# Zanue/EndoDAV

Hardware: AMD Instinct MI355X
Metric: depth frames/sec (518x518, T=8 clip) (higher is better)
Workload: dtype f32

## Files before the change

### endodav_amd/_lib.py

```python
from __future__ import annotations

import ctypes as C
import os
from typing import Optional

_HERE = os.path.dirname(os.path.abspath(__file__))
LIB_PATH = os.environ.get("EDV_LIB_PATH") or os.path.join(_HERE, "lib", "libendodav_hip.so")
ABI_VERSION = 12

LORA_TYPES = {"none": 0, "lora": 1, "dvlora": 2, "ssb": 3, "dash": 4}
ACT_NONE, ACT_GELU, ACT_RELU, ACT_SIGMOID, ACT_SIGMOID_NEG = 0, 1, 2, 3, 4


class EdvConfig(C.Structure):

    _fields_ = [
        ("abi_version", C.c_int32),
        ("embed_dim", C.c_int32),
        ("depth", C.c_int32),
        ("num_heads", C.c_int32),
        ("taps", C.c_int32 * 4),
        ("features", C.c_int32),
        ("out_channels", C.c_int32 * 4),
        ("image_h", C.c_int32),
        ("image_w", C.c_int32),
        ("num_frames", C.c_int32),
        ("pos_tokens", C.c_int32),
        ("lora_type", C.c_int32),
        ("lora_rank", C.c_int32),
        ("include_cls_token", C.c_int32),
        ("conv_head", C.c_int32),
        ("inv_sigmoid", C.c_int32),
        ("out_sigmoid", C.c_int32),
        ("temporal_lora", C.c_int32),
        ("dash_active", C.c_int32),
        ("use_clstoken", C.c_int32),
        ("residual_mask", C.c_uint32),
        ("use_bn", C.c_int32),
        ("pe_rope", C.c_int32),
    ]

# ... 43 lines not shown
    "edv_backward": (C.c_int, [C.c_void_p, C.c_uint64, _fp, C.POINTER(C.c_void_p), C.c_void_p]),
    "edv_grad_bind_flat": (C.c_int, [C.c_void_p, _i32, C.POINTER(C.c_char_p), C.POINTER(_i64), _fp, _i64, C.POINTER(_i64)]),
    "edv_grad": (C.c_int, [C.c_void_p, C.c_char_p, C.POINTER(C.c_void_p), C.POINTER(_i64)]),
    "edv_grad_copy": (C.c_int, [C.c_void_p, C.c_char_p, _fp, _i64, C.c_void_p]),
    "edv_attn_spatial_x6_workspace": (C.c_size_t, [_i32, _i32, _i32]),
    "edv_attn_spatial_x6": (C.c_int, [_fp, _fp, _i32, _i32, _i32, _fp, C.c_size_t, C.c_void_p]),
    "edv_attn_spatial_bwd_workspace": (C.c_size_t, [_i32, _i32, _i32]),
    "edv_attn_spatial_bwd": (C.c_int, [_fp, _fp, _fp, _fp, _fp, _fp, _i32, _i32, _i32, _fp, C.c_size_t, C.c_void_p]),
    "edv_layernorm_bwd": (C.c_int, [_fp, _fp, _fp, _fp, _i64, _i32, C.c_float, _i32, C.c_void_p]),
    "edv_ew_bwd": (C.c_int, [_fp, _fp, _fp, _fp, _i64, _i32, C.c_void_p]),
    "edv_geglu_bwd": (C.c_int, [_fp, _fp, _fp, _i64, _i32, C.c_void_p]),
    "edv_transpose_scale": (C.c_int, [_fp, _fp, _fp, _i32, _i32, C.c_void_p]),
    "edv_lora_grads_workspace": (C.c_size_t, [_i64, _i32, _i32, _i32]),
    "edv_lora_grads": (C.c_int, [_fp, _fp, _i64, _i32, _i32, _i32, _fp, _fp, _fp, _fp, C.c_float, _fp, _fp, C.c_size_t, _fp, _fp, _fp, _fp, C.c_void_p]),
    "edv_bilinear_bwd": (C.c_int, [_fp, _fp, _i32, _i32, _i32, _i32, _i32, _i32, _i32, C.c_void_p]),
    "edv_dot_channels_bwd": (C.c_int, [_fp, _fp, _fp, _fp, _fp, _fp, _i64, _i32, _i32, C.c_void_p]),
    "edv_conv3x3_wgrad_workspace": (C.c_size_t, [_i32, _i32, _i32, _i32, _i32]),
    "edv_conv3x3_wgrad": (C.c_int, [_fp, _fp, _fp, _i32, _i32, _i32, _i32, _i32, _fp, C.c_size_t, _i32, C.c_void_p]),
    "edv_colsum_workspace": (C.c_size_t, [_i32]),
    "edv_colsum_rows": (C.c_int, [_fp, _fp, _i64, _i32, _fp, C.c_size_t, _fp, _i32, C.c_void_p]),
    "edv_colsum_batch_workspace": (C.c_size_t, [_i32, C.POINTER(_i64), C.POINTER(_i32)]),
    "edv_colsum_batch": (C.c_int, [_i32, C.POINTER(C.c_void_p), C.POINTER(_i64), C.POINTER(_i64), C.POINTER(_i32), C.POINTER(_i32), C.POINTER(C.c_void_p),
                                   C.POINTER(C.c_void_p), C.POINTER(_i32), _fp, C.c_size_t, C.c_void_p]),
    "edv_groupnorm_bwd": (C.c_int, [_fp, _fp, _fp, _fp, _fp, _fp, _i32, _i32, _i32, _i32, _i32, C.c_void_p]),
    "edv_attn_temporal_bwd": (C.c_int, [_fp, _fp, _fp, _i32, _i32, _i32, _i32, _i32, C.c_void_p]),
    "edv_pack_conv3x3_bwd": (C.c_int, [_fp, _fp, _i32, _i32, C.c_void_p]),
    "edv_conv3x3_s2_bwd": (C.c_int, [_fp, _fp, _fp, _i32, _i32, _i32, _i32, _i32, C.c_void_p]),
    "edv_dilate2": (C.c_int, [_fp, _fp, _i32, _i32, _i32, _i32, C.c_void_p]),
    "edv_pixel_unshuffle": (C.c_int, [_fp, _fp, _i32, _i32, _i32, _i32, _i32, C.c_void_p]),
    "edv_attn_temporal": (C.c_int, [_fp, _fp, _i32, _i32, _i32, _i32, _i32, C.c_void_p]),
    "edv_groupnorm_workspace": (C.c_size_t, [_i32, _i32, _i32]),
    "edv_groupnorm": (C.c_int, [_fp, _fp, _fp, _fp, _fp, _i32, _i32, _i32, _i32, _f32, _fp, C.c_size_t, C.c_void_p]),
    "edv_geglu": (C.c_int, [_fp, _fp, _i64, _i32, C.c_void_p]),
    "edv_rope_qk": (C.c_int, [_fp, _fp, _i32, _i32, _i32, _i32, _i32, C.c_void_p]),
    "edv_trainer_loss_workspace": (C.c_size_t, [_i32, _i32, _i32]),
    "edv_trainer_loss": (C.c_int, [C.c_void_p, _i32, _i32, _i32, C.c_void_p, _fp, C.c_void_p, _fp, C.c_size_t, C.c_void_p]),
    "edv_debug_fill_lds": (C.c_int, [C.c_float, C.c_void_p]),
    "edv_bilinear": (C.c_int, [_fp, _fp, _i32, _i32, _i32, _i32, _i32, _i32, C.c_void_p]),
    "edv_dot_channels": (C.c_int, [_fp, _fp, _fp, _fp, _i64, _i32, _i32, C.c_void_p]),
    "edv_patchify": (C.c_int, [_fp, _fp, _i32, _i32, _i32, _i32, _i32, C.c_void_p]),
    "edv_bicubic_pos": (C.c_int, [_fp, _fp, _i32, _i32, _i32, _i32, _f64, _f64, C.c_void_p]),
    "edv_resize_bicubic": (C.c_int, [_fp, _fp, _i32, _i32, _i32, _i32, _i32, C.c_void_p]),
    "edv_stitch_workspace": (C.c_size_t, []),
    "edv_stitch_fit": (C.c_int, [_fp, _i32, _i32, _fp, _i32, _i32, _fp, _fp, C.c_size_t, C.c_void_p]),
    "edv_stitch_apply": (C.c_int, [_fp, _i32, _i32, _fp, _fp, _fp, _i32, _i32, C.c_void_p]),
    "edv_photometric_loss_workspace": (C.c_size_t, [_i32, _i32, _i32, _i32]),
    "edv_photometric_loss": (C.c_int, [_fp, C.POINTER(C.c_void_p), C.POINTER(_i32), C.POINTER(_i32), _i32, _i32, _i32, _i32, _fp, _fp, _fp, _fp, _f32, _f32, _f32,
                                       _fp, C.POINTER(C.c_void_p), _fp, C.c_size_t, C.c_void_p]),
    "edv_fold_lora": (C.c_int, [_fp, _fp, _fp, _fp, _fp, _f32, _fp, _i32, _i32, _i32, C.c_void_p]),
}


KERNEL_CLASSES = {"linear": 0, "conv3x3": 1, "attn_spatial": 2, "attn_temporal": 3, "layernorm": 4, "other": 5, "linear_encoder": 6,
                  "groupnorm": 7, "bilinear": 8, "geglu": 9, "dot_channels": 10, "patchify": 11, "attn_spatial_bwd": 12}
HBM_CLASSES = ("layernorm", "groupnorm", "bilinear", "geglu", "dot_channels", "patchify")


class EdvError(RuntimeError):
    pass


_lib: Optional[C.CDLL] = None


def load() -> C.CDLL:
    global _lib
# ... 2 lines not shown
    if not os.path.exists(LIB_PATH):
        raise EdvError(
            f"{LIB_PATH} is missing: build it with `make` (hipcc --offload-arch=gfx950) or "
            "`python -c 'import __graft_entry__ as g; g.build()'`.  There is no CPU fallback."
        )
    lib = C.CDLL(LIB_PATH)
    for name, (res, args) in SIGNATURES.items():
        fn = getattr(lib, name)
        fn.restype = res
        fn.argtypes = args
    got = lib.edv_abi_version()
    if got != ABI_VERSION:
        raise EdvError(f"libendodav_hip ABI {got} != binding ABI {ABI_VERSION}")
    _lib = lib
    return lib


def check(status: int, what: str = "") -> None:
    if status != 0:
        msg = load().edv_last_error()
        raise EdvError(f"{what}: {msg.decode() if msg else 'unknown error'}")


def ptr(t) -> int:
    return 0 if t is None else t.data_ptr()


class TrainerLossInputs(C.Structure):
    _fields_ = [("color", C.c_void_p * 4), ("color_nb", C.c_void_p * 2), ("K", C.c_void_p), ("invK", C.c_void_p), ("T", C.c_void_p * 2),
                ("refined", (C.c_void_p * 2) * 4), ("registration", (C.c_void_p * 2) * 4), ("transform", (C.c_void_p * 2) * 4), ("mask", C.c_void_p * 2),
                ("position", (C.c_void_p * 2) * 4), ("disp", C.c_void_p * 4), ("disp_h", C.c_int32 * 4), ("disp_w", C.c_int32 * 4)]


class TrainerLossWeights(C.Structure):
    _fields_ = [("disparity_smoothness", C.c_float), ("transform_constraint", C.c_float), ("transform_smoothness", C.c_float), ("depth_reproj", C.c_float),
                ("depth_flow", C.c_float), ("tune_temporal", C.c_int32), ("min_depth", C.c_float), ("max_depth", C.c_float)]


class TrainerLossGrads(C.Structure):
    _fields_ = [("disp", C.c_void_p * 4), ("refined", (C.c_void_p * 2) * 4), ("transform", (C.c_void_p * 2) * 4), ("K", C.c_void_p), ("invK", C.c_void_p),
                ("T", C.c_void_p * 2)]


def stream_ptr(device=None) -> int:
    import torch

    return torch.cuda.current_stream(device).cuda_stream
```

### endodav_amd/csrc/api.hip

```cpp
#include "../../include/endodav_hip.h"
#include <vector>

#include "ops.hpp"

using namespace edv;

extern "C" {

int edv_layernorm(const float *x_dev, const float *w_dev, const float *b_dev, float *y_dev, int64_t rows, int32_t dim, float eps,
                  const float *pe_dev, int32_t rows_per_frame, int32_t T, void *stream) {
    return layernorm(x_dev, identity_map(), w_dev, b_dev, y_dev, identity_map(), rows, dim, eps, pe_dev, rows_per_frame, T, (hipStream_t)stream);
}

size_t edv_gemm_workspace(void) { return gemm_workspace() * sizeof(float); }
int edv_gemm(const float *A_dev, const float *W_dev, float *C_dev, int64_t M, int32_t N, int32_t K, const float *bias_dev, int32_t act,
             const float *gamma_dev, const float *R_dev, float *workspace_dev, size_t workspace_bytes, void *stream) {
    GemmDesc g;
    g.A = A_dev; g.lda = K; g.W = W_dev; g.ldw = K; g.C = C_dev; g.ldc = N; g.M = M; g.N = N; g.K = K;
    g.bias = bias_dev; g.act = act; g.gamma = gamma_dev; g.R1 = R_dev; g.ldr1 = N;
    g.ws = workspace_dev; g.ws_floats = workspace_bytes / sizeof(float);
    EDV_CHECK(act >= ACT_NONE && act <= ACT_RELU, "act must be 0, 1 or 2");
    return gemm(g, (hipStream_t)stream);
}

size_t edv_gemm_x6_planes_bytes(int32_t N, int32_t K) { return N > 0 && K > 0 ? gemm_x6_planes_bytes(N, K) : 0; }

int edv_gemm_x6_split(const float *W_dev, void *planes_dev, int32_t N, int32_t K, void *stream) {
    return gemm_x6_split(W_dev, planes_dev, N, K, (hipStream_t)stream);
}

int edv_gemm_x6(const float *A_dev, const void *planes_dev, float *C_dev, int64_t M, int32_t N, int32_t K, const float *bias_dev, int32_t act,
                const float *gamma_dev, const float *R_dev, float *workspace_dev, size_t workspace_bytes, void *stream) {
    GemmDesc g;
// ... 139 lines not shown
    return groupnorm_bwd(x_dev, stats_dev, w_dev, dy_dev, sums_dev, dx_dev, F, P, C, groups, accumulate != 0, (hipStream_t)stream);
}
int edv_attn_temporal_bwd(const float *qkv_dev, const float *dout_dev, float *dqkv_dev, int32_t B, int32_t T, int32_t P, int32_t C, int32_t heads,
                          void *stream) {
    return attn_temporal_bwd(qkv_dev, dout_dev, dqkv_dev, B, T, P, C, heads, (hipStream_t)stream);
}
int edv_pack_conv3x3_bwd(const float *w_dev, float *wpacked_dev, int32_t Cout, int32_t Cin, void *stream) {
    return pack_conv3x3_bwd(w_dev, wpacked_dev, Cout, Cin, (hipStream_t)stream);
}
int edv_conv3x3_s2_bwd(const float *dy_dev, const float *wpacked_dev, float *dx_dev, int32_t F, int32_t H, int32_t W, int32_t Cin, int32_t Cout,
                       void *stream) {
    return conv3x3_s2_bwd(dy_dev, wpacked_dev, dx_dev, F, H, W, Cin, Cout, (hipStream_t)stream);
}
int edv_dilate2(const float *dy_dev, float *z_dev, int32_t F, int32_t H, int32_t W, int32_t C, void *stream) {
    return dilate2(dy_dev, z_dev, F, H, W, C, (hipStream_t)stream);
}
int edv_pixel_unshuffle(const float *dy_dev, float *A_dev, int32_t F, int32_t h, int32_t w, int32_t C, int32_t s, void *stream) {
    return pixel_unshuffle(dy_dev, A_dev, F, h, w, C, s, (hipStream_t)stream);
}

int edv_attn_temporal(const float *qkv_dev, float *out_dev, int32_t B, int32_t T, int32_t P, int32_t C, int32_t heads, void *stream) {
    return attn_temporal(qkv_dev, out_dev, B, T, P, C, heads, (hipStream_t)stream);
}

int edv_rope_qk(float *qkv_dev, const float *table_dev, int32_t B, int32_t T, int32_t P, int32_t C, int32_t transpose, void *stream) {
    return rope_qk(qkv_dev, table_dev, B, T, P, C, transpose != 0, (hipStream_t)stream);
}

size_t edv_groupnorm_workspace(int32_t F, int32_t P, int32_t C) { return groupnorm_workspace(F, P, C) * sizeof(float); }

int edv_groupnorm(const float *x_dev, const float *w_dev, const float *b_dev, float *y_dev, float *stats_dev, int32_t F, int32_t P, int32_t C,
                  int32_t groups, float eps, float *workspace_dev, size_t workspace_bytes, void *stream) {
    return groupnorm(x_dev, w_dev, b_dev, y_dev, stats_dev, F, P, C, groups, eps, (hipStream_t)stream, workspace_dev, workspace_bytes / sizeof(float));
}

namespace edv {
namespace {
__global__ __launch_bounds__(256) void fill_lds_kernel(float value, float *sink) {
    extern __shared__ float lds_all[];
    for (int i = threadIdx.x; i < 160 * 256; i += 256) lds_all[i] = value;
    __syncthreads();
    if (sink && lds_all[(threadIdx.x * 97) % (160 * 256)] != value) *sink = 1.f;
}
}
}
int edv_debug_fill_lds(float value, void *stream) {
    int dev = 0, cus = 0;
    EDV_HIP(hipGetDevice(&dev));
    EDV_HIP(hipDeviceGetAttribute(&cus, hipDeviceAttributeMultiprocessorCount, dev));
    EDV_HIP(hipFuncSetAttribute(reinterpret_cast<const void *>(edv::fill_lds_kernel), hipFuncAttributeMaxDynamicSharedMemorySize, 160 * 1024));
    EDV_LAUNCH(edv::fill_lds_kernel, dim3((unsigned)(8 * cus)), dim3(256), 160 * 1024, (hipStream_t)stream, value, (float *)nullptr);
    EDV_LAUNCH_OK();
    return 0;
}

int edv_geglu(const float *x_dev, float *y_dev, int64_t M, int32_t inner, void *stream) { return geglu(x_dev, y_dev, M, inner, (hipStream_t)stream); }

int edv_bilinear(const float *x_dev, float *y_dev, int32_t F, int32_t H, int32_t W, int32_t C, int32_t OH, int32_t OW, void *stream) {
    return bilinear(x_dev, y_dev, F, H, W, C, OH, OW, ACT_NONE, (hipStream_t)stream);
}

int edv_dot_channels(const float *x_dev, const float *w_dev, const float *b_dev, float *y_dev, int64_t M, int32_t C, int32_t act, void *stream) {
    EDV_CHECK(act == ACT_NONE || act == ACT_RELU || act == ACT_SIGMOID || act == ACT_SIGMOID_NEG, "act must be 0, 2, 3 or 4");
    return dot_channels(x_dev, w_dev, b_dev, y_dev, M, C, act, (hipStream_t)stream);
}

// ... 76 lines not shown
```

### endodav_amd/csrc/engine_forward.hip

```cpp
#include "engine.hpp"

namespace {

struct OnStream {
    Run &r;
    const hipStream_t st;
    float *const skws;
    const int F;
    OnStream(Run &run, hipStream_t s, float *ws) : r(run), st(run.st), skws(run.skws), F(run.F) { r.st = s; r.skws = ws; }
    ~OnStream() { r.st = st; r.skws = skws; r.F = F; }
};

struct Forward : Run {
    using Run::Run;
    std::string rb_suffix;
    int enc_F = 0, enc_f0 = 0;
    bool stagger_record = false;
    float *tap[4], *tapcls[4] = {nullptr, nullptr, nullptr, nullptr}, *pj[4], *lv[4], *rn[4], *path[5], *readout = nullptr, *fbias = nullptr;

    int pos_table(const float **out) {
        const float *pos;
        EDV_TRY(param("pretrained.pos_embed", &pos, 3));
        const int Npos = cfg.pos_tokens - 1;
        const int npatch = ntok - 1;
        if (npatch == Npos && cfg.image_h == cfg.image_w) {
            *out = pos;
            return 0;
        }
        const int S = (int)std::lround(std::sqrt((double)Npos));
        EDV_CHECK(S * S == Npos, "pos_embed grid is not square");
        float *tab;
        EDV_TRY(wsbuf("pos_eff", (size_t)ntok * D, &tab));
        const double sh = ((double)ph + 0.1) / std::sqrt((double)Npos), sw = ((double)pw + 0.1) / std::sqrt((double)Npos);
        EDV_CHECK((int)std::floor(S * sh) == ph && (int)std::floor(S * sw) == pw, "pos-embed resample size mismatch");
        if (c0) EDV_TRY(copy_f32(pos, tab, D, st));
        EDV_TRY(bicubic_pos(pos + D, tab + (size_t)c0 * D, S, D, ph, pw, (float)(1.0 / sh), (float)(1.0 / sw), st));
        c->launches += 2;
        *out = tab;
        return 0;
    }

    int snapshot(const std::string &name, const float *src, size_t n) {
        if (c->capture) {
            float *dst;
            EDV_TRY(wsbuf("stage." + name, n, &dst));
            EDV_TRY(copy_f32(src, dst, (long long)n, st));
            c->stages[name] = {dst, n};
        }
        return 0;
    }

    int motion_module(int m, float *x, int P, int C, const float *extra = nullptr) {
        const std::string p = "head.motion_modules." + std::to_string(m) + ".temporal_transformer";
        const std::string tb = p + ".transformer_blocks.0";
        const long long M = (long long)F * P;
        float *gn, *h, *hn, *qkv3, *att, *ff1, *ff2, *stats;
        const std::string sc_ = m == 1 ? "mmb." : "mm.";
        const std::string tg = c->train ? "mm" + std::to_string(m) + "." : sc_;
        float *hs[4];
        const float *xin = x;
        EDV_TRY(wsbuf(sc_ + "gn", (size_t)M * C, &gn));
        EDV_TRY(wsbuf(tg + "h", (size_t)M * C, &h));
        hs[0] = hs[1] = hs[2] = hs[3] = h;
        if (c->train) {
            float *xc;
            EDV_TRY(wsbuf(tg + "xin", (size_t)M * C, &xc));
            EDV_TRY(copy_f32(x, xc, M * C, st));
            xin = xc;
            for (int k = 1; k < 4; ++k) EDV_TRY(wsbuf(tg + "h" + std::to_string(k), (size_t)M * C, &hs[k]));
        }
        EDV_TRY(wsbuf(sc_ + "hn", (size_t)M * C, &hn));
        EDV_TRY(wsbuf(sc_ + "att", (size_t)M * C, &att));
        EDV_TRY(wsbuf(tg + "ff1", (size_t)M * 8 * C, &ff1));
        EDV_TRY(wsbuf(c->train ? tg + "ff2" : sc_ + "ff2", (size_t)M * 4 * C, &ff2));
        EDV_TRY(wsbuf(tg + "stats", (size_t)F * 32 * 2, &stats));
        const float *w, *b;
        EDV_TRY(param(p + ".norm.weight", &w));
        EDV_TRY(param(p + ".norm.bias", &b));
        float *gnpart = nullptr;
        size_t gnpart_n = 0;
        if ((long long)F * P * C >= 1500000ll) {
            gnpart_n = groupnorm_workspace(F, P, C);
            EDV_TRY(wsbuf(sc_ + "gnpart", gnpart_n, &gnpart));
        }
        {
            HbmScope b_(c, KC_GROUPNORM, st, 8.0 * (double)M * C);
            EDV_TRY(groupnorm(xin, w, b, gn, stats, F, P, C, 32, 1e-6f, st, gnpart, gnpart_n));
        }
// ... 612 lines not shown
```

### endodav_amd/csrc/norms.hip

```cpp
#include <cstdlib>

#include "ops.hpp"

namespace edv {
namespace {

using f32x4 = __attribute__((ext_vector_type(4))) float;
constexpr int LN_MAXV = 4;

template <int R, int NV>
__global__ __launch_bounds__(256) void layernorm_kernel(const float *__restrict__ x, RowMap in_map, const float *__restrict__ w,
                                                         const float *__restrict__ b, float *y, RowMap out_map, long long rows,
                                                         int dim, float eps, const float *__restrict__ pe, int rows_per_frame, int T, int act,
                                                         int accumulate) {
    const int lane = threadIdx.x & 63;
    const long long row0 = ((long long)blockIdx.x * 4 + (threadIdx.x >> 6)) * R;
    if (row0 >= rows) return;
    const int nv = dim >> 2;
    f32x4 v[R][NV];
    float s[R];
#pragma unroll
    for (int k = 0; k < R; ++k) {
        const long long row = row0 + k < rows ? row0 + k : rows - 1;
        const float *xr = x + in_map(row) * dim;
// ... 182 lines not shown
    EDV_CHECK(x && w && b && y, "null operand");
    EDV_CHECK(act == ACT_NONE || act == ACT_GELU, "layernorm act must be none or gelu");
    EDV_CHECK(rows > 0, "empty problem");
    EDV_CHECK(dim % 4 == 0 && dim <= 256 * LN_MAXV, "dim must be a multiple of 4 and <= 1024");
    EDV_CHECK(!pe || (rows_per_frame > 0 && T > 0), "pe needs rows_per_frame and T");
    static const int forced = [] {
        const char *e = getenv("EDV_LN_ROWS");
        return e ? atoi(e) : 0;
    }();
    int R = 1;
    if (forced == 1 || forced == 2 || forced == 4) R = forced;
    if (dim > 512 && R > 2) R = 2;
    const long long blocks = (rows + 4 * R - 1) / (4 * R);
    EDV_CHECK(blocks < (1ll << 31), "grid");
    const int rpf = rows_per_frame > 0 ? rows_per_frame : 1, TT = T > 0 ? T : 1, acc = accumulate ? 1 : 0;
#define EDV_LN_LAUNCH(RR, NVV)                                                                                                                  \
    EDV_LAUNCH((layernorm_kernel<RR, NVV>), dim3((unsigned)blocks), dim3(256), 0, st, x, in_map, w, b, y, out_map, rows, dim, eps, pe, rpf, TT, \
                       act, acc)
    if (dim <= 512) {
        if (R == 4) EDV_LN_LAUNCH(4, 2);
        else if (R == 2) EDV_LN_LAUNCH(2, 2);
        else EDV_LN_LAUNCH(1, 2);
    } else {
        if (R == 2) EDV_LN_LAUNCH(2, 4);
        else EDV_LN_LAUNCH(1, 4);
    }
#undef EDV_LN_LAUNCH
    EDV_LAUNCH_OK();
    return 0;
}

size_t groupnorm_workspace(int F, int P, int C) { return (size_t)F * ((P + GN_ROWS - 1) / GN_ROWS) * 2 * C; }

int groupnorm(const float *x, const float *w, const float *b, float *y, float *stats, int F, int P, int C, int groups, float eps, hipStream_t st, float *part,
              size_t part_floats) {
    EDV_CHECK(x && w && b && y && stats, "null operand");
    EDV_CHECK(F > 0 && P > 0 && C > 0 && groups > 0 && C % groups == 0 && C % 4 == 0, "shape");
    EDV_CHECK(F <= 65535, "grid");
    const int nch = (P + GN_ROWS - 1) / GN_ROWS;
    if (part && C <= 1024 && nch <= 65535) {
        EDV_CHECK(groupnorm_workspace(F, P, C) <= part_floats && (uintptr_t)part % 16 == 0, "groupnorm workspace too small (groupnorm_workspace)");
        EDV_LAUNCH(groupnorm_partial_kernel, dim3(nch, F), dim3(256), 0, st, x, part, P, C, nch);
        EDV_LAUNCH_OK();
        EDV_LAUNCH(groupnorm_finish_kernel, dim3(groups, F), dim3(64), 0, st, part, stats, P, C, groups, nch, eps);
        EDV_LAUNCH_OK();
    } else {
        EDV_LAUNCH(groupnorm_stats_kernel, dim3(groups, F), dim3(256), 0, st, x, stats, P, C, groups, eps);
        EDV_LAUNCH_OK();
    }
    EDV_CHECK(C <= 1024, "groupnorm: at most 1024 channels");
    const int rpp = 256 / (C >> 2);
    int chunks = (P + 4 * rpp - 1) / (4 * rpp);
    chunks = chunks < 1 ? 1 : (chunks > 2048 ? 2048 : chunks);
    EDV_LAUNCH(groupnorm_apply_kernel, dim3((unsigned)chunks, (unsigned)F), dim3(256), 0, st, x, stats, w, b, y, P, C, groups);
    EDV_LAUNCH_OK();
    return 0;
}

}
```

### endodav_amd/csrc/ops.hpp

```cpp
#pragma once
#include "common.hpp"

namespace edv {

enum { ACT_NONE = 0, ACT_GELU = 1, ACT_RELU = 2, ACT_SIGMOID = 3, ACT_SIGMOID_NEG = 4 };
enum { LOAD_DENSE = 0, LOAD_CONV3 = 1 };
enum { STORE_ROWS = 0, STORE_SHUFFLE = 1 };

struct GemmDesc {
    const float *A = nullptr;
    int lda = 0;
    RowMap a_map{0, 0, 0};
    const float *W = nullptr;
    int ldw = 0;
    float *C = nullptr;
    int ldc = 0;
    RowMap c_map{0, 0, 0};
    long long M = 0;
    int N = 0, K = 0;
    const float *bias = nullptr;
    int act = ACT_NONE;
    const float *gamma = nullptr;
    const float *R1 = nullptr;
    int ldr1 = 0;
// ... 9 lines not shown
    int geglu = 0;
    int ps_s = 0, ps_C = 0, ps_h = 0, ps_w = 0;
    float *ws = nullptr;
    size_t ws_floats = 0;
    const void *Wx6 = nullptr;
};
int gemm(const GemmDesc &d, hipStream_t st);
size_t gemm_x6_planes_bytes(int N, int K);
int gemm_x6_split(const float *W, void *planes, int N, int K, hipStream_t st);
bool gemm_x6_supported(const GemmDesc &d);
int gemm_x6(const GemmDesc &d, hipStream_t st);
size_t gemm_workspace();
size_t gemm_counter_bytes();
bool gemm_dma_supported(const GemmDesc &d);
bool gemm_geglu_supported(const GemmDesc &d);
int pack_geglu(const float *w, const float *b, float *wi, float *bi, int N, int K, hipStream_t st);
int gemm_dma(const GemmDesc &d, hipStream_t st);
bool conv_dma_supported(const GemmDesc &d);
int conv_dma(const GemmDesc &d, hipStream_t st);
const char *gemm_kernel_name(const GemmDesc &d);

size_t attn_spatial_workspace(int F, int N, int heads, bool x6 = false);
int attn_spatial(const float *qkv, float *out, int F, int N, int heads, float *ws, size_t ws_floats, hipStream_t st, float *lse = nullptr, bool x6 = false);
size_t attn_spatial_bwd_workspace(int F, int N, int heads);
int attn_spatial_bwd(const float *qkv, const float *out, const float *dout, const float *lse, float *delta, float *dqkv, int F, int N, int heads, float *ws,
                     size_t ws_floats, hipStream_t st);
int attn_temporal(const float *qkv, float *out, int B, int T, int P, int C, int heads, hipStream_t st);
int geglu(const float *x, float *y, long long M, int inner, hipStream_t st);
int rope_qk(float *qkv, const float *table, int B, int T, int P, int C, bool transpose, hipStream_t st);

int layernorm(const float *x, RowMap in_map, const float *w, const float *b, float *y, RowMap out_map, long long rows, int dim,
              float eps, const float *pe, int rows_per_frame, int T, hipStream_t st, int act = ACT_NONE, bool accumulate = false);
size_t groupnorm_workspace(int F, int P, int C);
int groupnorm(const float *x, const float *w, const float *b, float *y, float *stats, int F, int P, int C, int groups, float eps, hipStream_t st,
              float *part = nullptr, size_t part_floats = 0);

int patchify(const float *x, float *cols, int F, int H, int W, int ih, int iw, hipStream_t st, int ld = 588)  ;
int bilinear(const float *x, float *y, int F, int H, int W, int C, int OH, int OW, int act, hipStream_t st, const float *add = nullptr);
int dot_channels(const float *x, const float *w, const float *b, float *y, long long M, int C, int act, hipStream_t st);
int cls_rows(const float *cls, const float *pos, float *tokens, int F, int ntok, int D, hipStream_t st);
int sigmoid_inplace(float *x, long long n, hipStream_t st);
int resize_bicubic(const float *x, float *y, int NP, int H, int W, int OH, int OW, hipStream_t st);
size_t stitch_workspace();
int stitch_fit(const float *disp, int ih, int iw, const float *tail, int fh, int fw, float *st, void *ws, size_t ws_bytes, hipStream_t stream);
int stitch_apply(const float *disp, int ih, int iw, const float *st, float *tail, float *out_new, int fh, int fw, hipStream_t stream);
int bicubic_pos(const float *grid, float *out, int S, int D, int oh, int ow, float scale_h, float scale_w, hipStream_t st);

int pack_conv3x3(const float *w, float *out, int Cout, int Cin, hipStream_t st);
int pack_convT(const float *w, float *wout, const float *b, float *bout, int Cin, int Cout, int s, hipStream_t st);
int copy_f32(const float *src, float *dst, long long n, hipStream_t st);
int fold_lora(const float *W, const float *A, const float *B, const float *U, const float *V, float scale, float *out, int nout, int nin,
              int r, hipStream_t st);
int fold_ssb(const float *W, const float *a, const float *b, float *out, int nout, int nin, hipStream_t st);
int fold_bn(float *w, const float *b, const float *gamma, const float *beta, const float *mean, const float *var, float eps, float *bout, int nout, int K,
            hipStream_t st);
int fold_dash(const float *Utop, const float *idx, const float *Vtop, float *inout, int nout, int nin, int r, hipStream_t st);

int layernorm_bwd(const float *x, RowMap xmap, const float *w, const float *dy, RowMap dymap, float *dx, RowMap dxmap, long long rows, int dim, float eps,
                  bool accumulate, hipStream_t st);
int ew_bwd(const float *d, const float *src, const float *add, float *out, long long n, int mode, hipStream_t st);
int sigmoid_bwd(const float *g, const float *s, float *out, long long n, hipStream_t st);
int geglu_bwd(const float *x, const float *dy, float *dx, long long M, int inner, hipStream_t st);
int transpose_scale(const float *W, int ldw, const float *gamma, float *Wt, int N, int K, hipStream_t st);
int skinny_xwt(const float *X, long long M, int K, int ldx, const float *Wr, int r, float *T, hipStream_t st);
constexpr int TALL_SPLITS = 64;
size_t tall_tn_workspace(int N, int r);
int tall_tn(const float *Y, int ldy, const float *T, long long M, int N, int r, float scale, const float *rowscale, float *part, float *out, hipStream_t st);
int lora_grad_finalize(const float *dBp, const float *dApT, const float *A, const float *Bm, const float *U, const float *V, float *dA, float *dB, float *dU,
// ... 73 lines not shown
```

### include/endodav_hip.h

```cpp
#ifndef ENDODAV_HIP_H
#define ENDODAV_HIP_H

#include <stddef.h>
#include <stdint.h>

#ifdef __cplusplus
extern "C" {
#endif

#define EDV_ABI_VERSION 12

enum edv_lora_type { EDV_LORA_NONE = 0, EDV_LORA_LORA = 1, EDV_LORA_DVLORA = 2, EDV_LORA_SSB = 3, EDV_LORA_DASH = 4 };

typedef struct edv_config {
    int32_t abi_version;
    int32_t embed_dim;
    int32_t depth;
    int32_t num_heads;
    int32_t taps[4];
    int32_t features;
    int32_t out_channels[4];
    int32_t image_h, image_w;
    int32_t num_frames;
    int32_t pos_tokens;
    int32_t lora_type;
    int32_t lora_rank;
    int32_t include_cls_token;
    int32_t conv_head;
    int32_t inv_sigmoid;
    int32_t out_sigmoid;
    int32_t temporal_lora;
    int32_t dash_active;
    int32_t use_clstoken;
    uint32_t residual_mask;
    int32_t use_bn;
    int32_t pe_rope;
} edv_config;

typedef struct edv_ctx edv_ctx;

int edv_abi_version(void);
const char *edv_last_error(void);
int edv_create(const edv_config *cfg, edv_ctx **out);
// ... 31 lines not shown
size_t edv_gemm_x6_planes_bytes(int32_t N, int32_t K);
int edv_gemm_x6_split(const float *W_dev, void *planes_dev, int32_t N, int32_t K, void *stream);
int edv_gemm_x6(const float *A_dev, const void *planes_dev, float *C_dev, int64_t M, int32_t N, int32_t K, const float *bias_dev, int32_t act,
                const float *gamma_dev, const float *R_dev, float *workspace_dev, size_t workspace_bytes, void *stream);

int edv_pack_geglu(const float *w_dev, const float *b_dev, float *wi_dev, float *bi_dev, int32_t N, int32_t K, void *stream);
int edv_gemm_geglu(const float *A_dev, const float *Wi_dev, const float *bi_dev, float *C_dev, int64_t M, int32_t N, int32_t K, void *stream);

int edv_conv3x3(const float *x_dev, const float *wpacked_dev, const float *bias_dev, float *y_dev, int32_t F, int32_t H, int32_t W,
                int32_t Cin, int32_t Cout, int32_t stride, int32_t pre_relu, int32_t post_relu, const float *R1_dev,
                const float *R2_dev, void *stream);
int edv_conv3x3_ws(const float *x_dev, const float *wpacked_dev, const float *bias_dev, float *y_dev, int32_t F, int32_t H, int32_t W,
                   int32_t Cin, int32_t Cout, int32_t stride, int32_t pre_relu, int32_t post_relu, const float *R1_dev,
                   const float *R2_dev, float *workspace_dev, size_t workspace_bytes, void *stream);
int edv_pack_conv3x3(const float *w_dev, float *wpacked_dev, int32_t Cout, int32_t Cin, void *stream);

size_t edv_attn_spatial_workspace(int32_t F, int32_t N, int32_t heads);
int edv_attn_spatial(const float *qkv_dev, float *out_dev, int32_t F, int32_t N, int32_t heads, float *workspace_dev,
                     size_t workspace_bytes, float *lse_dev, void *stream);
size_t edv_attn_spatial_x6_workspace(int32_t F, int32_t N, int32_t heads);
int edv_attn_spatial_x6(const float *qkv_dev, float *out_dev, int32_t F, int32_t N, int32_t heads, float *workspace_dev, size_t workspace_bytes,
                        void *stream);
size_t edv_attn_spatial_bwd_workspace(int32_t F, int32_t N, int32_t heads);
int edv_attn_spatial_bwd(const float *qkv_dev, const float *out_dev, const float *dout_dev, const float *lse_dev, float *delta_dev,
                         float *dqkv_dev, int32_t F, int32_t N, int32_t heads, float *workspace_dev, size_t workspace_bytes, void *stream);

int edv_attn_temporal(const float *qkv_dev, float *out_dev, int32_t B, int32_t T, int32_t P, int32_t C, int32_t heads, void *stream);

int edv_rope_qk(float *qkv_dev, const float *table_dev, int32_t B, int32_t T, int32_t P, int32_t C, int32_t transpose, void *stream);

size_t edv_groupnorm_workspace(int32_t F, int32_t P, int32_t C);
int edv_groupnorm(const float *x_dev, const float *w_dev, const float *b_dev, float *y_dev, float *stats_dev ,
                  int32_t F, int32_t P, int32_t C, int32_t groups, float eps, float *workspace_dev, size_t workspace_bytes, void *stream);

int edv_geglu(const float *x_dev, float *y_dev, int64_t M, int32_t inner, void *stream);

int edv_debug_fill_lds(float value, void *stream);

int edv_bilinear(const float *x_dev, float *y_dev, int32_t F, int32_t H, int32_t W, int32_t C, int32_t OH, int32_t OW, void *stream);

int edv_dot_channels(const float *x_dev, const float *w_dev, const float *b_dev, float *y_dev, int64_t M, int32_t C, int32_t act, void *stream);

int edv_patchify(const float *x_dev, float *cols_dev, int32_t F, int32_t H, int32_t W, int32_t ih, int32_t iw, void *stream);

int edv_conv_transpose(const float *x_dev, const float *w_dev, const float *b_dev, float *wpack_dev, float *bpack_dev, float *y_dev, int32_t F, int32_t h,
              int32_t w, int32_t C, int32_t s, void *stream);

int edv_bicubic_pos(const float *grid_dev, float *out_dev, int32_t S, int32_t D, int32_t oh, int32_t ow, double scale_h, double scale_w, void *stream);

int edv_resize_bicubic(const float *x_dev, float *y_dev, int32_t planes, int32_t H, int32_t W, int32_t OH, int32_t OW, void *stream);

size_t edv_stitch_workspace(void);
int edv_stitch_fit(const float *disp_dev, int32_t ih, int32_t iw, const float *tail_dev, int32_t fh, int32_t fw, float *st_dev, void *workspace_dev,
                   size_t workspace_bytes, void *stream);
int edv_stitch_apply(const float *disp_dev, int32_t ih, int32_t iw, const float *st_dev, float *tail_dev, float *new_dev, int32_t fh, int32_t fw,
                     void *stream);

int edv_fold_lora(const float *W_dev, const float *A_dev, const float *B_dev, const float *U_dev, const float *V_dev, float scale, float *out_dev,
                  int32_t nout, int32_t nin, int32_t r, void *stream);

int edv_set_train(edv_ctx *ctx, int32_t on);
int edv_set_grad_scope(edv_ctx *ctx, int32_t encoder_factors, int32_t temporal_factors, int32_t head_convs, int32_t residual_blocks);
int edv_set_bias_grads(edv_ctx *ctx, int32_t encoder_biases, int32_t head_biases);
int edv_generation(const edv_ctx *ctx, uint64_t *generation);
int edv_backward(edv_ctx *ctx, uint64_t generation, const float *disp0_dev, const float *const grad_disp_dev[4], void *stream);
int edv_grad_bind_flat(edv_ctx *ctx, int32_t n, const char *const *names, const int64_t *numels, float *flat_dev, int64_t flat_floats,
// ... 71 lines not shown
```

Before: 1077.

## Fuse temporal motion module into a single MFMA kernel per pixel tile

Adds a fused HIP kernel that runs the whole temporal transformer motion module (groupnorm apply, proj_in, two temporal attention blocks with layernorm and positional encoding, GEGLU feed-forward, proj_out and residual) for 64-channel, 8-head blocks in registers using fp32 MFMA. Only groupnorm statistics stay in a separate launch, which removes many intermediate global-memory round trips and kernel launches in inference. It is enabled by default for non-training runs without RoPE, and adds a new ABI entry point. The cost is heavy register use and redundant weight loads per wave.

After: 1082, median of 6. Within noise of the previous version (+0.5%).

```diff
diff --git a/endodav_amd/_lib.py b/endodav_amd/_lib.py
--- a/endodav_amd/_lib.py
+++ b/endodav_amd/_lib.py
@@ -6,7 +6,7 @@
 
 _HERE = os.path.dirname(os.path.abspath(__file__))
 LIB_PATH = os.environ.get("EDV_LIB_PATH") or os.path.join(_HERE, "lib", "libendodav_hip.so")
-ABI_VERSION = 12
+ABI_VERSION = 13
 
 LORA_TYPES = {"none": 0, "lora": 1, "dvlora": 2, "ssb": 3, "dash": 4}
 ACT_NONE, ACT_GELU, ACT_RELU, ACT_SIGMOID, ACT_SIGMOID_NEG = 0, 1, 2, 3, 4
@@ -116,6 +116,9 @@
     "edv_groupnorm_workspace": (C.c_size_t, [_i32, _i32, _i32]),
     "edv_groupnorm": (C.c_int, [_fp, _fp, _fp, _fp, _fp, _i32, _i32, _i32, _i32, _f32, _fp, C.c_size_t, C.c_void_p]),
     "edv_geglu": (C.c_int, [_fp, _fp, _i64, _i32, C.c_void_p]),
+    "edv_motion_module_fused_supported": (C.c_int, [_i32, _i32, _i32]),
+    "edv_motion_module_fused_workspace": (C.c_size_t, [_i32, _i32, _i32]),
+    "edv_motion_module_fused": (C.c_int, [_fp, _fp, C.c_void_p, _fp, C.c_size_t, _i32, _i32, _i32, C.c_void_p]),
     "edv_rope_qk": (C.c_int, [_fp, _fp, _i32, _i32, _i32, _i32, _i32, C.c_void_p]),
     "edv_trainer_loss_workspace": (C.c_size_t, [_i32, _i32, _i32]),
     "edv_trainer_loss": (C.c_int, [C.c_void_p, _i32, _i32, _i32, C.c_void_p, _fp, C.c_void_p, _fp, C.c_size_t, C.c_void_p]),
@@ -184,6 +187,13 @@
                 ("position", (C.c_void_p * 2) * 4), ("disp", C.c_void_p * 4), ("disp_h", C.c_int32 * 4), ("disp_w", C.c_int32 * 4)]
 
 
+class MotionParams(C.Structure):
+    _fields_ = [("gn_w", C.c_void_p), ("gn_b", C.c_void_p), ("proj_in_w", C.c_void_p), ("proj_in_b", C.c_void_p), ("ln_w", C.c_void_p * 2),
+                ("ln_b", C.c_void_p * 2), ("pe", C.c_void_p * 2), ("qkv_w", C.c_void_p * 2), ("out_w", C.c_void_p * 2), ("out_b", C.c_void_p * 2),
+                ("ffn_w", C.c_void_p), ("ffn_b", C.c_void_p), ("ff0_w", C.c_void_p), ("ff0_b", C.c_void_p), ("ff2_w", C.c_void_p), ("ff2_b", C.c_void_p),
+                ("proj_out_w", C.c_void_p), ("proj_out_b", C.c_void_p)]
+
+
 class TrainerLossWeights(C.Structure):
     _fields_ = [("disparity_smoothness", C.c_float), ("transform_constraint", C.c_float), ("transform_smoothness", C.c_float), ("depth_reproj", C.c_float),
                 ("depth_flow", C.c_float), ("tune_temporal", C.c_int32), ("min_depth", C.c_float), ("max_depth", C.c_float)]
diff --git a/endodav_amd/csrc/api.hip b/endodav_amd/csrc/api.hip
--- a/endodav_amd/csrc/api.hip
+++ b/endodav_amd/csrc/api.hip
@@ -1,4 +1,5 @@
 #include "../../include/endodav_hip.h"
+#include <cstring>
 #include <vector>
 
 #include "ops.hpp"
@@ -204,6 +205,21 @@
 int edv_groupnorm(const float *x_dev, const float *w_dev, const float *b_dev, float *y_dev, float *stats_dev, int32_t F, int32_t P, int32_t C,
                   int32_t groups, float eps, float *workspace_dev, size_t workspace_bytes, void *stream) {
     return groupnorm(x_dev, w_dev, b_dev, y_dev, stats_dev, F, P, C, groups, eps, (hipStream_t)stream, workspace_dev, workspace_bytes / sizeof(float));
+}
+
+int edv_motion_module_fused_supported(int32_t T, int32_t C, int32_t heads) { return motion_fused_supported(T, C, heads) ? 1 : 0; }
+
+size_t edv_motion_module_fused_workspace(int32_t B, int32_t T, int32_t P) {
+    return B > 0 && T > 0 && P > 0 ? motion_module_fused_workspace(B * T, P) * sizeof(float) : 0;
+}
+
+int edv_motion_module_fused(float *x_dev, const float *extra_dev, const edv_motion_params *params, float *workspace_dev, size_t workspace_bytes, int32_t B,
+                            int32_t T, int32_t P, void *stream) {
+    EDV_CHECK(params, "null argument");
+    static_assert(sizeof(edv_motion_params) == sizeof(MotionFusedParams), "edv_motion_params mirrors MotionFusedParams");
+    MotionFusedParams q;
+    memcpy(&q, params, sizeof(q));
+    return motion_module_fused(x_dev, extra_dev, q, workspace_dev, workspace_bytes / sizeof(float), B, T, P, (hipStream_t)stream);
 }
 
 namespace edv {
diff --git a/endodav_amd/csrc/engine_forward.hip b/endodav_amd/csrc/engine_forward.hip
--- a/endodav_amd/csrc/engine_forward.hip
+++ b/endodav_amd/csrc/engine_forward.hip
@@ -50,10 +50,42 @@
         return 0;
     }
 
+    int motion_module_fused_path(const std::string &p, const std::string &tb, int m, float *x, int P, const float *extra) {
+        MotionFusedParams q;
+        EDV_TRY(param(p + ".norm.weight", &q.gn_w));
+        EDV_TRY(param(p + ".norm.bias", &q.gn_b));
+        EDV_TRY(param(p + ".proj_in.weight", &q.proj_in_w));
+        EDV_TRY(param(p + ".proj_in.bias", &q.proj_in_b));
+        for (int a = 0; a < 2; ++a) {
+            const std::string ab = tb + ".attention_blocks." + std::to_string(a), nb = tb + ".norms." + std::to_string(a);
+            EDV_TRY(param(nb + ".weight", &q.ln_w[a]));
+            EDV_TRY(param(nb + ".bias", &q.ln_b[a]));
+            EDV_TRY(param(ab + ".pos_encoder.pe", &q.pe[a]));
+            EDV_TRY(packedw(ab + ".qkv", &q.qkv_w[a]));
+            EDV_TRY(param(ab + ".to_out.0.weight", &q.out_w[a]));
+            EDV_TRY(param(ab + ".to_out.0.bias", &q.out_b[a]));
+        }
+        EDV_TRY(param(tb + ".ff_norm.weight", &q.ffn_w));
+        EDV_TRY(param(tb + ".ff_norm.bias", &q.ffn_b));
+        EDV_TRY(param(tb + ".ff.net.0.proj.weight", &q.ff0_w));
+        EDV_TRY(param(tb + ".ff.net.0.proj.bias", &q.ff0_b));
+        EDV_TRY(lin_w(tb + ".ff.net.2", &q.ff2_w));
+        EDV_TRY(param(tb + ".ff.net.2.bias", &q.ff2_b));
+        EDV_TRY(param(p + ".proj_out.weight", &q.proj_out_w));
+        EDV_TRY(param(p + ".proj_out.bias", &q.proj_out_b));
+        const size_t nws = motion_module_fused_workspace(F, P);
+        float *ws;
+        EDV_TRY(wsbuf((m == 1 ? "mmb." : "mm.") + std::string("fused"), nws, &ws));
+        Bracket b_(c, KC_ATTN_TEMPORAL, st);
+        return motion_module_fused(x, extra, q, ws, nws, B, T, P, st, &c->launches);
+    }
+
     int motion_module(int m, float *x, int P, int C, const float *extra = nullptr) {
         const std::string p = "head.motion_modules." + std::to_string(m) + ".temporal_transformer";
         const std::string tb = p + ".transformer_blocks.0";
         const long long M = (long long)F * P;
+        static const bool mm_fused = env_flag("EDV_MM_FUSED", true);
+        if (mm_fused && !c->train && !cfg.pe_rope && motion_fused_supported(T, C, 8)) return motion_module_fused_path(p, tb, m, x, P, extra);
         float *gn, *h, *hn, *qkv3, *att, *ff1, *ff2, *stats;
         const std::string sc_ = m == 1 ? "mmb." : "mm.";
         const std::string tg = c->train ? "mm" + std::to_string(m) + "." : sc_;
diff --git a/endodav_amd/csrc/motion_fused.hip b/endodav_amd/csrc/motion_fused.hip
--- /dev/null
+++ b/endodav_amd/csrc/motion_fused.hip
@@ -0,0 +1,223 @@
+#include "ops.hpp"
+
+namespace edv {
+namespace {
+
+using f32x4 = __attribute__((ext_vector_type(4))) float;
+using f32x16 = __attribute__((ext_vector_type(16))) float;
+
+__device__ __forceinline__ f32x4 ld4(const float *p) { return *reinterpret_cast<const f32x4 *>(p); }
+
+template <int KB>
+__device__ __forceinline__ f32x16 lin32(f32x16 acc, const float *__restrict__ wr, const f32x16 (&xin)[KB]) {
+#pragma unroll
+    for (int kb = 0; kb < KB; ++kb) {
+#pragma unroll
+        for (int q = 0; q < 4; ++q) {
+            const f32x4 w4 = ld4(wr + 32 * kb + 8 * q);
+#pragma unroll
+            for (int e = 0; e < 4; ++e) acc = __builtin_amdgcn_mfma_f32_32x32x2f32(w4[e], xin[kb][4 * q + e], acc, 0, 0, 0);
+        }
+    }
+    return acc;
+}
+
+__device__ __forceinline__ f32x16 feat32(const float *__restrict__ v) {
+    f32x16 o;
+#pragma unroll
+    for (int q = 0; q < 4; ++q) {
+        const f32x4 b4 = ld4(v + 8 * q);
+#pragma unroll
+        for (int e = 0; e < 4; ++e) o[4 * q + e] = b4[e];
+    }
+    return o;
+}
+
+__device__ __forceinline__ float hsum16(const f32x16 v) {
+    return (((v[0] + v[1]) + (v[2] + v[3])) + ((v[4] + v[5]) + (v[6] + v[7]))) + (((v[8] + v[9]) + (v[10] + v[11])) + ((v[12] + v[13]) + (v[14] + v[15])));
+}
+
+__device__ __forceinline__ void ln64(const f32x16 (&in)[2], f32x16 (&out)[2], const float *__restrict__ w, const float *__restrict__ b,
+                                     const float *__restrict__ pe, int h, float eps) {
+    float s = hsum16(in[0]) + hsum16(in[1]);
+    s += __shfl_xor(s, 32, 64);
+    const float mean = s * (1.0f / 64.0f);
+    const f32x16 d0 = in[0] - mean, d1 = in[1] - mean;
+    float q = hsum16(d0 * d0) + hsum16(d1 * d1);
+    q += __shfl_xor(q, 32, 64);
+    const float rstd = rsqrtf(q * (1.0f / 64.0f) + eps);
+    out[0] = d0 * rstd * feat32(w + 4 * h) + feat32(b + 4 * h);
+    out[1] = d1 * rstd * feat32(w + 32 + 4 * h) + feat32(b + 32 + 4 * h);
+    if (pe) {
+        out[0] += feat32(pe);
+        out[1] += feat32(pe + 32);
+    }
+}
+
+template <int T>
+__device__ __forceinline__ f32x16 attn_block(const f32x16 q, const f32x16 k, const f32x16 v, float scale) {
+    float s[4][T];
+#pragma unroll
+    for (int j = 0; j < T; ++j) {
+#pragma unroll
+        for (int hh = 0; hh < 4; ++hh) {
+            float kk[4];
+#pragma unroll
+            for (int e = 0; e < 4; ++e) kk[e] = j ? __shfl_xor(k[4 * hh + e], j, 64) : k[4 * hh + e];
+            s[hh][j] = (q[4 * hh] * kk[0] + q[4 * hh + 1] * kk[1]) + (q[4 * hh + 2] * kk[2] + q[4 * hh + 3] * kk[3]);
+        }
+    }
+    float inv[4];
+#pragma unroll
+    for (int hh = 0; hh < 4; ++hh) {
+        float mx = -INFINITY;
+#pragma unroll
+        for (int j = 0; j < T; ++j) {
+            s[hh][j] = (s[hh][j] + __shfl_xor(s[hh][j], 32, 64)) * scale;
+            mx = fmaxf(mx, s[hh][j]);
+        }
+        float sum = 0.f;
+#pragma unroll
+        for (int j = 0; j < T; ++j) {
+            s[hh][j] = expf(s[hh][j] - mx);
+            sum += s[hh][j];
+        }
+        inv[hh] = 1.0f / sum;
+    }
+    f32x16 o;
+#pragma unroll
+    for (int i = 0; i < 16; ++i) o[i] = s[i >> 2][0] * v[i];
+#pragma unroll
+    for (int j = 1; j < T; ++j) {
+#pragma unroll
+        for (int i = 0; i < 16; ++i) o[i] += s[i >> 2][j] * __shfl_xor(v[i], j, 64);
+    }
+#pragma unroll
+    for (int i = 0; i < 16; ++i) o[i] *= inv[i >> 2];
+    return o;
+}
+
+template <int T>
+__global__ __launch_bounds__(256, 2) void motion_fused_kernel(float *x, const float *__restrict__ extra, const MotionFusedParams p,
+                                                            const float *__restrict__ stats, int P, int tiles_per_clip, int ntiles) {
+    constexpr int PPT = 32 / T;
+    constexpr int C = 64;
+    const int lane = threadIdx.x & 63, n = lane & 31, h = lane >> 5;
+    const int tile = blockIdx.x * 4 + (threadIdx.x >> 6);
+    if (tile >= ntiles) return;
+    const int b = tile / tiles_per_clip, tc = tile - b * tiles_per_clip;
+    const int t = n % T;
+    int pix = tc * PPT + n / T;
+    const bool valid = pix < P;
+    if (!valid) pix = P - 1;
+    const long long frame = (long long)b * T + t;
+    const long long off = (frame * P + pix) * C + 4 * h;
+
+    f32x16 a[2];
+#pragma unroll
+    for (int q = 0; q < 8; ++q) {
+        const f32x4 v = ld4(x + off + 8 * q);
+        const f32x4 ms = ld4(stats + (frame * 32 + 4 * q + 2 * h) * 2);
+        const f32x4 gw = ld4(p.gn_w + 8 * q + 4 * h), gb = ld4(p.gn_b + 8 * q + 4 * h);
+        a[q >> 2][4 * (q & 3) + 0] = (v[0] - ms[0]) * (ms[1] * gw[0]) + gb[0];
+        a[q >> 2][4 * (q & 3) + 1] = (v[1] - ms[0]) * (ms[1] * gw[1]) + gb[1];
+        a[q >> 2][4 * (q & 3) + 2] = (v[2] - ms[2]) * (ms[3] * gw[2]) + gb[2];
+        a[q >> 2][4 * (q & 3) + 3] = (v[3] - ms[2]) * (ms[3] * gw[3]) + gb[3];
+    }
+    const int wrow = n * C + 4 * h;
+    f32x16 hres[2], hn[2];
+#pragma unroll
+    for (int ob = 0; ob < 2; ++ob) hres[ob] = lin32<2>(feat32(p.proj_in_b + 32 * ob + 4 * h), p.proj_in_w + 32 * ob * C + wrow, a);
+
+    const float scale = 0.35355339059327373f;
+#pragma unroll 1
+    for (int ab = 0; ab < 2; ++ab) {
+        ln64(hres, hn, p.ln_w[ab], p.ln_b[ab], p.pe[ab] + t * C + 4 * h, h, 1e-5f);
+        const float *__restrict__ wq = p.qkv_w[ab] + wrow;
+        f32x16 o[2];
+#pragma unroll
+        for (int blk = 0; blk < 2; ++blk) {
+            f32x16 z = {0.f, 0.f, 0.f, 0.f, 0.f, 0.f, 0.f, 0.f, 0.f, 0.f, 0.f, 0.f, 0.f, 0.f, 0.f, 0.f};
+            const f32x16 qq = lin32<2>(z, wq + (32 * blk) * C, hn);
+            const f32x16 kk = lin32<2>(z, wq + (64 + 32 * blk) * C, hn);
+            const f32x16 vv = lin32<2>(z, wq + (128 + 32 * blk) * C, hn);
+            o[blk] = attn_block<T>(qq, kk, vv, scale);
+        }
+#pragma unroll
+        for (int ob = 0; ob < 2; ++ob) hres[ob] += lin32<2>(feat32(p.out_b[ab] + 32 * ob + 4 * h), p.out_w[ab] + 32 * ob * C + wrow, o);
+    }
+
+    ln64(hres, hn, p.ffn_w, p.ffn_b, nullptr, h, 1e-5f);
+    f32x16 y[2];
+#pragma unroll
+    for (int ob = 0; ob < 2; ++ob) y[ob] = feat32(p.ff2_b + 32 * ob + 4 * h);
+#pragma unroll 1
+    for (int c = 0; c < 8; ++c) {
+        const f32x16 val = lin32<2>(feat32(p.ff0_b + 32 * c + 4 * h), p.ff0_w + (32 * c) * C + wrow, hn);
+        const f32x16 gate = lin32<2>(feat32(p.ff0_b + 256 + 32 * c + 4 * h), p.ff0_w + (256 + 32 * c) * C + wrow, hn);
+        f32x16 g[1];
+#pragma unroll
+        for (int i = 0; i < 16; ++i) g[0][i] = val[i] * gelu_erf(gate[i]);
+#pragma unroll
+        for (int ob = 0; ob < 2; ++ob) y[ob] = lin32<1>(y[ob], p.ff2_w + (32 * ob + n) * (4 * C) + 32 * c + 4 * h, g);
+    }
+#pragma unroll
+    for (int ob = 0; ob < 2; ++ob) hres[ob] += y[ob];
+
+#pragma unroll
+    for (int ob = 0; ob < 2; ++ob) y[ob] = lin32<2>(feat32(p.proj_out_b + 32 * ob + 4 * h), p.proj_out_w + 32 * ob * C + wrow, hres);
+    if (!valid) return;
+#pragma unroll
+    for (int q = 0; q < 8; ++q) {
+        f32x4 r = ld4(x + off + 8 * q);
+        if (extra) r += ld4(extra + off + 8 * q);
+#pragma unroll
+        for (int e = 0; e < 4; ++e) r[e] += y[q >> 2][4 * (q & 3) + e];
+        *reinterpret_cast<f32x4 *>(x + off + 8 * q) = r;
+    }
+}
+
+}
+
+bool motion_fused_supported(int T, int C, int heads) { return C == 64 && heads == 8 && (T == 2 || T == 4 || T == 8 || T == 16); }
+
+int motion_fused(float *x, const float *extra, const MotionFusedParams &p, const float *stats, int B, int T, int P, hipStream_t st) {
+    EDV_CHECK(x && stats, "null operand");
+    EDV_CHECK(B > 0 && P > 0, "empty problem");
+    EDV_CHECK(motion_fused_supported(T, 64, 8), "unsupported clip length (motion_fused_supported)");
+    const float *const *pp = reinterpret_cast<const float *const *>(&p);
+    for (size_t i = 0; i < sizeof(p) / sizeof(const float *); ++i) EDV_CHECK(pp[i] && (uintptr_t)pp[i] % 16 == 0, "null or misaligned parameter");
+    EDV_CHECK((uintptr_t)x % 16 == 0 && (uintptr_t)extra % 16 == 0 && (uintptr_t)stats % 16 == 0, "operands must be 16-byte aligned");
+    const int ppt = 32 / T;
+    const long long tpc = (P + ppt - 1) / ppt, ntiles = tpc * B;
+    EDV_CHECK(ntiles < (1ll << 31) - 4, "grid");
+    const dim3 grid((unsigned)((ntiles + 3) / 4)), block(256);
+#define EDV_MM_LAUNCH(TT) EDV_LAUNCH(motion_fused_kernel<TT>, grid, block, 0, st, x, extra, p, stats, P, (int)tpc, (int)ntiles)
+    if (T == 2) EDV_MM_LAUNCH(2);
+    else if (T == 4) EDV_MM_LAUNCH(4);
+    else if (T == 8) EDV_MM_LAUNCH(8);
+    else EDV_MM_LAUNCH(16);
+#undef EDV_MM_LAUNCH
+    EDV_LAUNCH_OK();
+    return 0;
+}
+
+size_t motion_module_fused_workspace(int F, int P) {
+    return (size_t)F * 32 * 2 + (groupnorm_two_stage_pays(F, P, 64) ? groupnorm_workspace(F, P, 64) : 0);
+}
+
+int motion_module_fused(float *x, const float *extra, const MotionFusedParams &p, float *ws, size_t ws_floats, int B, int T, int P, hipStream_t st,
+                        int *launches) {
+    EDV_CHECK(x && ws, "null operand");
+    EDV_CHECK(B > 0 && T > 0 && P > 0 && (long long)B * T <= 65535, "shape");
+    EDV_CHECK(motion_fused_supported(T, 64, 8), "unsupported clip length (motion_fused_supported)");
+    const int F = B * T;
+    EDV_CHECK(ws_floats >= motion_module_fused_workspace(F, P) && (uintptr_t)ws % 16 == 0, "workspace too small or misaligned (motion_module_fused_workspace)");
+    const bool two = groupnorm_two_stage_pays(F, P, 64);
+    EDV_TRY(groupnorm_stats(x, ws, F, P, 64, 32, 1e-6f, st, two ? ws + (size_t)F * 64 : nullptr, two ? groupnorm_workspace(F, P, 64) : 0));
+    EDV_TRY(motion_fused(x, extra, p, ws, B, T, P, st));
+    if (launches) *launches += two ? 3 : 2;
+    return 0;
+}
+
+}
diff --git a/endodav_amd/csrc/norms.hip b/endodav_amd/csrc/norms.hip
--- a/endodav_amd/csrc/norms.hip
+++ b/endodav_amd/csrc/norms.hip
@@ -238,9 +238,10 @@
 
 size_t groupnorm_workspace(int F, int P, int C) { return (size_t)F * ((P + GN_ROWS - 1) / GN_ROWS) * 2 * C; }
 
-int groupnorm(const float *x, const float *w, const float *b, float *y, float *stats, int F, int P, int C, int groups, float eps, hipStream_t st, float *part,
-              size_t part_floats) {
-    EDV_CHECK(x && w && b && y && stats, "null operand");
+bool groupnorm_two_stage_pays(int F, int P, int C) { return (long long)F * P * C >= 1500000ll; }
+
+int groupnorm_stats(const float *x, float *stats, int F, int P, int C, int groups, float eps, hipStream_t st, float *part, size_t part_floats) {
+    EDV_CHECK(x && stats, "null operand");
     EDV_CHECK(F > 0 && P > 0 && C > 0 && groups > 0 && C % groups == 0 && C % 4 == 0, "shape");
     EDV_CHECK(F <= 65535, "grid");
     const int nch = (P + GN_ROWS - 1) / GN_ROWS;
@@ -254,6 +255,13 @@
         EDV_LAUNCH(groupnorm_stats_kernel, dim3(groups, F), dim3(256), 0, st, x, stats, P, C, groups, eps);
         EDV_LAUNCH_OK();
     }
+    return 0;
+}
+
+int groupnorm(const float *x, const float *w, const float *b, float *y, float *stats, int F, int P, int C, int groups, float eps, hipStream_t st, float *part,
+              size_t part_floats) {
+    EDV_CHECK(x && w && b && y && stats, "null operand");
+    EDV_TRY(groupnorm_stats(x, stats, F, P, C, groups, eps, st, part, part_floats));
     EDV_CHECK(C <= 1024, "groupnorm: at most 1024 channels");
     const int rpp = 256 / (C >> 2);
     int chunks = (P + 4 * rpp - 1) / (4 * rpp);
diff --git a/endodav_amd/csrc/ops.hpp b/endodav_amd/csrc/ops.hpp
--- a/endodav_amd/csrc/ops.hpp
+++ b/endodav_amd/csrc/ops.hpp
@@ -65,8 +65,28 @@
 int layernorm(const float *x, RowMap in_map, const float *w, const float *b, float *y, RowMap out_map, long long rows, int dim,
               float eps, const float *pe, int rows_per_frame, int T, hipStream_t st, int act = ACT_NONE, bool accumulate = false);
 size_t groupnorm_workspace(int F, int P, int C);
+bool groupnorm_two_stage_pays(int F, int P, int C);
 int groupnorm(const float *x, const float *w, const float *b, float *y, float *stats, int F, int P, int C, int groups, float eps, hipStream_t st,
               float *part = nullptr, size_t part_floats = 0);
+int groupnorm_stats(const float *x, float *stats, int F, int P, int C, int groups, float eps, hipStream_t st, float *part = nullptr, size_t part_floats = 0);
+
+struct MotionFusedParams {
+    const float *gn_w, *gn_b;
+    const float *proj_in_w, *proj_in_b;
+    const float *ln_w[2], *ln_b[2];
+    const float *pe[2];
+    const float *qkv_w[2];
+    const float *out_w[2], *out_b[2];
+    const float *ffn_w, *ffn_b;
+    const float *ff0_w, *ff0_b;
+    const float *ff2_w, *ff2_b;
+    const float *proj_out_w, *proj_out_b;
+};
+bool motion_fused_supported(int T, int C, int heads);
+int motion_fused(float *x, const float *extra, const MotionFusedParams &p, const float *stats, int B, int T, int P, hipStream_t st);
+size_t motion_module_fused_workspace(int F, int P);
+int motion_module_fused(float *x, const float *extra, const MotionFusedParams &p, float *ws, size_t ws_floats, int B, int T, int P, hipStream_t st,
+                        int *launches = nullptr);
 
 int patchify(const float *x, float *cols, int F, int H, int W, int ih, int iw, hipStream_t st, int ld = 588)  ;
 int bilinear(const float *x, float *y, int F, int H, int W, int C, int OH, int OW, int act, hipStream_t st, const float *add = nullptr);
diff --git a/include/endodav_hip.h b/include/endodav_hip.h
--- a/include/endodav_hip.h
+++ b/include/endodav_hip.h
@@ -8,7 +8,7 @@
 extern "C" {
 #endif
 
-#define EDV_ABI_VERSION 12
+#define EDV_ABI_VERSION 13
 
 enum edv_lora_type { EDV_LORA_NONE = 0, EDV_LORA_LORA = 1, EDV_LORA_DVLORA = 2, EDV_LORA_SSB = 3, EDV_LORA_DASH = 4 };
 
@@ -106,6 +106,23 @@
 size_t edv_groupnorm_workspace(int32_t F, int32_t P, int32_t C);
 int edv_groupnorm(const float *x_dev, const float *w_dev, const float *b_dev, float *y_dev, float *stats_dev ,
                   int32_t F, int32_t P, int32_t C, int32_t groups, float eps, float *workspace_dev, size_t workspace_bytes, void *stream);
+
+typedef struct {
+    const float *gn_w, *gn_b;
+    const float *proj_in_w, *proj_in_b;
+    const float *ln_w[2], *ln_b[2];
+    const float *pe[2];
+    const float *qkv_w[2];
+    const float *out_w[2], *out_b[2];
+    const float *ffn_w, *ffn_b;
+    const float *ff0_w, *ff0_b;
+    const float *ff2_w, *ff2_b;
+    const float *proj_out_w, *proj_out_b;
+} edv_motion_params;
+int edv_motion_module_fused_supported(int32_t T, int32_t C, int32_t heads);
+size_t edv_motion_module_fused_workspace(int32_t B, int32_t T, int32_t P);
+int edv_motion_module_fused(float *x_dev, const float *extra_dev , const edv_motion_params *params, float *workspace_dev,
+                            size_t workspace_bytes, int32_t B, int32_t T, int32_t P, void *stream);
 
 int edv_geglu(const float *x_dev, float *y_dev, int64_t M, int32_t inner, void *stream);
 
```
